# PaddleCV-SIG/MedicalSeg

Measured on AMD Instinct MI355X. Metric: 3D-voxels/sec fwd+bwd, VNet 128^3 fp32, higher is better.
Workload: dtype f32

## Files before the change

### medicalseg_amd/csrc/msk_common.h

```cpp
#pragma once
#include <hip/hip_runtime.h>
#include <hip/hip_ext.h>

#include <cstdint>
#include <cstdio>
#include <cstring>
#include <map>
#include <set>
#include <string>
#include <utility>
#include <vector>

#include "msegk.h"

struct msk_prof_entry {
  double total_ms = 0.0;
  long calls = 0;
};

struct msk_pending_event {
  hipEvent_t a, b;
  const char* tag;
};

// ... 4 lines not shown
  virtual int prepack(msk_ctx* ctx, const void* p, size_t bytes) = 0;
};

struct msk_ctx {
  int device = 0;
  hipStream_t stream = nullptr;
  std::string err;
  void* ws = nullptr;
  size_t ws_bytes = 0;
  void* ws2 = nullptr;
  size_t ws2_bytes = 0;
  void* ws3 = nullptr;
  size_t ws3_bytes = 0;
  long wbf_tin_groups = -1;
  long wbf_pad_min_voxels = 1L << 18;
  hipEvent_t t0 = nullptr, t1 = nullptr;
  hipEvent_t ev_xctx = nullptr;
  bool prof = false;
  std::map<std::string, msk_prof_entry> prof_map;
  std::vector<msk_pending_event> prof_pending;
  std::vector<hipEvent_t> event_pool;
  std::vector<hipEvent_t> marks;
  std::set<std::string> tag_pool;
  bool prof_shapes = false;
  int conv_impl = 0;
  bool no_winograd = false;
  bool wbf = true;
  bool dst_split_done = false;
  bool stats_fused = false;
  bool wgrad_db_done = false;
  bool xform_written = false;
  std::set<const void*> xform_ok;
  bool conv_fp16 = false;
  int wbf_tin_map = 1;
  int wbf_mr4 = 1;
  int wbf_variant = -1;
  int halo_tile = -1;
  int wgrad_chunk = -1;
  char prof_prefix[48] = {0};
  long wgrad_async_max_m = 0;
  float* scalar_ring = nullptr;
  int scalar_next = 0;
  long scalar_served = 0;
  float* scalar_ring_side = nullptr;
  int scalar_next_side = 0;
  long scalar_served_side = 0;
  int wbf_tpb = 0;
  msk_pack_cache* wpack = nullptr;
  int wbf_pack_cache = 1;
  msk_pack_cache* spack = nullptr;
  int wbf_pack_lds = 1;
  int wbf_bpf = 1;
  int wbf_fused_sh = 1;
  int wbf_gemm_form = -1;
  int wbf_ks_blocks = 2;
  int noop_after_merge = 0;
  int wgrad_c1_wpc = 2;
  int eager_tail_main = 1;
  int prof_paused = 0;
  int prof_attach = 1;
  int small_pack_cache = 1;
  int wbf_prepack = 1;
  int ks_legacy = 0;
  int wgrad_fork = 1;
  int wbf_fused_bl = 2;
  int wbf_fuse = 1;
  int conv_split = 2;
  int bwd_fuse = -1;
  int foldn_wgs = 0;
  int wgrad_wino_rounds = 0;
  int wgrad_rounds = 8;
  int poison = -1;
  hipStream_t side = nullptr;
  void* ws_side = nullptr;
  size_t ws_side_bytes = 0;
  void* ws3_side = nullptr;
  size_t ws3_side_bytes = 0;
  hipEvent_t ev_fork = nullptr, ev_join = nullptr;
  hipEvent_t ev_late = nullptr;
  bool late_valid = false;
  const float* late_ptr = nullptr;
  size_t late_count = 0;
  float* late_alpha = nullptr;
  struct { float* param = nullptr; const float* grad = nullptr; float* velocity = nullptr; size_t count = 0;
           float lr = 0, momentum = 0, weight_decay = 0, grad_scale = 0; } late_piece;
  int late_split = 1;
  bool wgrad_async = false;
  bool side_dirty = false;
  hipEvent_t fork_event = nullptr;
  int fork_attach = 1;
  bool fork_recorded = false;
  void* stage[2] = {nullptr, nullptr};
  size_t stage_bytes[2] = {0, 0};
  hipEvent_t stage_ev[2] = {nullptr, nullptr};
  int stage_next = 0;
  void* comm = nullptr;
  void* comm_grad = nullptr;
  hipStream_t comm_stream = nullptr;
  hipEvent_t ev_comm_main = nullptr, ev_comm_side = nullptr, ev_comm_done = nullptr, ev_comm_back = nullptr;
  int c1_h2 = 1;
  int dst_split = 1;
  int wgrad_reduce_rows = 1;
  int ks_stats = 1;
  int ks_lds = 1;
  int ks_nr_max = 4;
  int wgrad_lds_pad = 0;
// ... 134 lines not shown
```

### medicalseg_amd/csrc/msk_conv_wbf.hip

```cpp
#include <type_traits>
#include "msk_pack.h"
#include "msk_wbf.h"
#ifndef WBF_TIN_SYNC
#define WBF_TIN_SYNC 1
#endif

#ifndef WBF_PROBE
#define WBF_PROBE 0
#endif
typedef _Float16 f16x8 __attribute__((ext_vector_type(8)));
typedef _Float16 f16x2 __attribute__((ext_vector_type(2)));

namespace {

constexpr int nxi_of(int K) { return K == 5 ? 8 : 6; }

__device__ __forceinline__ void split3_one(float x, unsigned short& hi, unsigned short& mid, unsigned short& lo) {
  hi = __builtin_bit_cast(unsigned short, (__bf16)x);
  const float r = x - __uint_as_float((unsigned)hi << 16);
  mid = __builtin_bit_cast(unsigned short, (__bf16)r);
  const float r2 = r - __uint_as_float((unsigned)mid << 16);
  lo = __builtin_bit_cast(unsigned short, (__bf16)r2);
}
__device__ __forceinline__ unsigned pack_f16_pair(float a, float b) {
// ... 566 lines not shown
    }
    if (WY) {
#pragma unroll
      for (int q = 0; q < 2; ++q) {
        float wx[8], wy[8], wz[8], ww[8];
#pragma unroll
        for (int j = 0; j < 4; ++j) {
          const float4 e = win[PADW + j][q];
          wx[j] = e.x; wy[j] = e.y; wz[j] = e.z; ww[j] = e.w;
        }
#pragma unroll
        for (int j = 4; j < 8; ++j) wx[j] = wy[j] = wz[j] = ww[j] = 0.f;
        tin_transform<1, K>(wx, v[q * 4 + 0]);
        tin_transform<1, K>(wy, v[q * 4 + 1]);
        tin_transform<1, K>(wz, v[q * 4 + 2]);
        tin_transform<1, K>(ww, v[q * 4 + 3]);
      }
#pragma unroll
      for (int xi = 0; xi < NXI; ++xi) store_xi<K, NP>(yb2 + t * tstep + (long)xi * b.y_xi, plane, v, xi, sc2);
    }
#pragma unroll
    for (int j = 0; j < KEEP; ++j) {
      win[j][0] = win[j + 4][0];
      win[j][1] = win[j + 4][1];
    }
#pragma unroll
    for (int j = 0; j < 4; ++j) {
      win[KEEP + j][0] = nxt[j][0];
      win[KEEP + j][1] = nxt[j][1];
    }
  }
  }
  if (want_cmax) wbf_cmax_commit(b.y_cmax, cg, cmx, true);
}

struct GemmArgs {
  const char* V;
  const char* U;
  float* M;
  int N, T, KC, CN, LD, LH, DP, HP;
  int tiles_d, tiles_h, ngrp, ksplit, kc_per;
  int tpb, nblk;
  long v_xi, v_plane;
  long u_xi;
  long m_xi;
};

__device__ __forceinline__ uint4 buf_load16(__amdgpu_buffer_rsrc_t r, unsigned lane_bytes, unsigned uniform_bytes) {
  return __builtin_bit_cast(uint4, __builtin_amdgcn_raw_buffer_load_b128(r, (int)lane_bytes, (int)uniform_bytes, 0));
}

typedef int i32x4 __attribute__((ext_vector_type(4)));
__device__ __forceinline__ void wbf_dma16(i32x4 rs, unsigned lds_addr, unsigned voff, unsigned soff) {
  asm volatile("s_mov_b32 m0, %0\n\ts_nop 0\n\tbuffer_load_dwordx4 %1, %2, %3 offen lds" ::"s"(lds_addr), "v"(voff), "s"(rs), "s"(soff) : "memory");
}

#define WBF_MFMA(acc, av, bv) \
  acc = __builtin_amdgcn_mfma_f32_32x32x16_bf16(__builtin_bit_cast(bf16x8, av), __builtin_bit_cast(bf16x8, bv), acc, 0, 0, 0)
#define WBF_MFMA_H(acc, av, bv) \
  acc = __builtin_amdgcn_mfma_f32_32x32x16_f16(__builtin_bit_cast(f16x8, av), __builtin_bit_cast(f16x8, bv), acc, 0, 0, 0)

template <int TH>
__device__ __forceinline__ void frag_pos(int r, int& a, int& b) {
  if (TH == 16) {
    if (r < 4) { a = 0; b = r; }
    else if (r < 12) { a = 0; b = r + 4; }
    else if (r < 16) { a = 0; b = r - 8; }
    else if (r < 20) { a = 1; b = r - 4; }
    else if (r < 28) { a = 1; b = r - 16; }
    else { a = 1; b = r - 28; }
  } else if (TH == 8) {
    if (r < 4) { a = 0; b = r; }
    else if (r < 12) { a = 1; b = r - 4; }
    else if (r < 16) { a = 0; b = r - 8; }
    else if (r < 20) { a = 3; b = r - 16; }
    else if (r < 28) { a = 2; b = r - 20; }
    else { a = 3; b = r - 24; }
  } else {
    a = r / TH;
    b = r % TH;
  }
}

template <int TH>
__device__ __forceinline__ void subfrag_pos(int g, int r, int& d, int& h) {
  if (TH == 8) { d = (g >> 1) * 4 + (g & 1) + 2 * (r >> 3); h = r & 7; }
  else { d = g / (TH / 16); h = (g % (TH / 16)) * 16 + r; }
}
#define WBF_MFMA16_H(acc, wv, av) \
  acc = __builtin_amdgcn_mfma_f32_16x16x32_f16(__builtin_bit_cast(f16x8, wv), __builtin_bit_cast(f16x8, av), acc, 0, 0, 0)

template <int MR, int WM, int WN, int TD, int TH, int K, int NP, int BPF = 1, int SH = 32>
__global__ void __launch_bounds__(WM * WN * 64)
wbf_gemm_k(GemmArgs a) {
  static_assert((WM * WN == 4 || WM * WN == 2) && WM * MR * 32 == TD * TH, "tile shape");
  static_assert(SH == 32 || (SH == 16 && NP == 2 && BPF == 1), "stage form");
  constexpr int CPS = SH == 16 ? 2 : 1;
  constexpr int NT = WM * WN * 64;
  constexpr int NXI = nxi_of(K), T2 = K * K, PADK = (K - 1) / 2;
  constexpr int HDt = TD + K - 1, HPt = TH + K - 1, NSLOT = HDt * HPt, NPL = 2 * NP, NIT = CPS * NPL * NSLOT, ROUNDS = (NIT + NT - 1) / NT;
  static_assert(SH == 32 || NSLOT % 16 == 0, "planes of the image start on a bank row (subfrag_pos)");
  __shared__ uint4 lds[ROUNDS * NT];

  const int tid = threadIdx.x;
  const int wave = __builtin_amdgcn_readfirstlane(tid >> 6), lane = tid & 63, li = lane & 31, lh = lane >> 5;
  const int wm = wave / WN, wn = wave % WN;

// ... 236 lines not shown

struct FusedArgs {
  GemmArgs g;
  float* dst;
  int dld;
  long dvn;
  int dvd, dvh, dvw;
  const float* bias;
  const float* prelu;
  int accumulate;
  const float* in_amax;
  const float* w_amax;
  int scaled;
  float* stat_partial;
  int per_xcd;
  int LW;
  float* st_lo;
  float* st_hi;
  int csplit;
  const float* acc_src;
};

struct WfRec {
  float n, mean, m2;
};
__device__ __forceinline__ WfRec wfrec_merge(WfRec a, WfRec b) {
  if (b.n == 0.f) return a;
  if (a.n == 0.f) return b;
  WfRec r;
  r.n = a.n + b.n;
  const float d = b.mean - a.mean, f = b.n / r.n;
  r.mean = a.mean + d * f;
  r.m2 = a.m2 + b.m2 + d * d * a.n * f;
  return r;
}

template <int K>
__device__ __forceinline__ void at_column(int xi, float& c0, float& c1, float& c2, float& c3) {
  const int last = K == 5 ? 7 : 5;
  c0 = xi == last ? 0.f : 1.f;
  if (xi == 0) { c1 = c2 = c3 = 0.f; return; }
  if (xi == last) { c1 = c2 = 0.f; c3 = 1.f; return; }
  const float sg = (xi & 1) ? 1.f : -1.f;
  const int pr = (xi - 1) >> 1;
  const float p = pr == 0 ? 1.f : (pr == 1 ? 2.f : 0.5f);
  c1 = sg * p;
  c2 = p * p;
  c3 = sg * p * p * p;
}

#ifndef WBF_FUSED_BPF
#define WBF_FUSED_BPF 3
#endif
template <int MR, int WM, int WN, int TD, int TH, int K, int NP, bool STATS, int BPF = (NP == 2 ? WBF_FUSED_BPF : 1), int BL = 0, int SH = 32>
__global__ void __launch_bounds__(WM * WN * 64, 2)
wbf_gemm_fused_k(FusedArgs f) {
  static_assert(WM * WN == 4 && WM * MR * 32 == TD * TH, "tile shape");
  static_assert(SH == 32 || (SH == 16 && BL == 2 && WN == 1 && NP == 2), "16x16x32: pipelined form, one column fragment");
  constexpr int NS16 = 2 * MR;
  const GemmArgs& a = f.g;
  constexpr int NT = WM * WN * 64;
  constexpr int NXI = nxi_of(K), T2 = K * K, PADK = (K - 1) / 2;
  constexpr int HDt = TD + K - 1, HPt = TH + K - 1, NSLOT = HDt * HPt, NPL = 2 * NP, NIT = NPL * NSLOT, ROUNDS = (NIT + NT - 1) / NT;
  constexpr int NBF = T2 * NP;
  constexpr int BROUNDS = (NBF + WM * WN - 1) / (WM * WN);
  static_assert(BL == 0 || NIT % 64 == 0, "weights through LDS: wave-granular tile");
  static_assert(BL != 1 || WN == 1, "B through LDS, whole stage: one column fragment");
  constexpr int PH = WN == 1 ? 4 : 5;
  constexpr int PQ_T[6] = {0, T2 * 1 / PH, T2 * 2 / PH, T2 * 3 / PH, PH > 4 ? T2 * 4 / PH : T2, T2};
  constexpr int PQ_FR = (T2 - PQ_T[PH - 1]) * NP * WN;
  constexpr int PQ_SLOT = PQ_FR * 64;
  static_assert(BL != 2 || (NP == 2 && WM * WN == 4 && WN <= 2 && PQ_T[1] * NP * WN >= 4), "pipelined form: fp16 x 2 pieces, four wavefronts");
  __shared__ uint4 lds[BL == 2 ? 2 * NIT + 2 * PQ_SLOT : (BL ? NIT + NBF * 64 : ROUNDS * NT)];

  const int tid = threadIdx.x;
  const int wave = __builtin_amdgcn_readfirstlane(tid >> 6), lane = tid & 63, li = lane & 31, lh = lane >> 5;
  const int wm = wave / WN, wn = wave % WN;

  int b = (blockIdx.x & 7) * f.per_xcd + (blockIdx.x >> 3);
  if ((int)(blockIdx.x >> 3) >= f.per_xcd || b >= a.nblk) return;
  const int tile_id = b;
  const int thi = b % a.tiles_h;
  b /= a.tiles_h;
  const int tdi = b % a.tiles_d;
  b /= a.tiles_d;
  const int t = b % a.T;
  const int n = b / a.T;

  unsigned voff[ROUNDS];
#pragma unroll
  for (int r = 0; r < ROUNDS; ++r) {
    int it = r * NT + tid;
    if (it >= NIT) it = 0;
    const int pk = it / NSLOT, slot = it - pk * NSLOT;
    const int row = slot / HPt, col = slot - row * HPt;
    voff[r] = (unsigned)(pk * a.v_plane + ((long)row * a.HP + col) * 16);
  }
  const char* vtile0 = a.V + ((long)(n * a.T + t) * a.KC) * NPL * a.v_plane +
                       ((long)(tdi * TD + 2 - PADK) * a.HP + thi * TH + 2 - PADK) * 16;
  const unsigned ulane = (unsigned)(lh * a.CN + wn * 32 + li) * 16u;
  const unsigned ustep = (unsigned)a.CN * 32u;
  const unsigned uchunk = (unsigned)NP * ustep;
  const unsigned utap = (unsigned)a.KC * uchunk;

  int arow[MR];
#pragma unroll
  for (int mr = 0; mr < MR; ++mr) {
    int fa, fb;
    frag_pos<TH>(li, fa, fb);
    arow[mr] = lh * NSLOT + ((wm * MR + mr) * (32 / TH) + fa) * HPt + fb;
  }

  f32x16 yo[4][MR];
#pragma unroll
  for (int i = 0; i < 4; ++i)
#pragma unroll
    for (int mr = 0; mr < MR; ++mr)
#pragma unroll
      for (int j = 0; j < 16; ++j) yo[i][mr][j] = 0.f;
  f32x4 yo16[4][NS16][2];
#pragma unroll
  for (int i = 0; i < 4; ++i)
#pragma unroll
    for (int s = 0; s < NS16; ++s)
#pragma unroll
      for (int ct = 0; ct < 2; ++ct) yo16[i][s][ct] = f32x4{0.f, 0.f, 0.f, 0.f};
  const int l16 = lane & 15, kq = lane >> 4;

  if constexpr (BL == 2) {
    const unsigned lds0 = (unsigned)(unsigned long)(__attribute__((address_space(3))) void*)lds;
    const int NS = NXI * a.KC;
    const unsigned voff_last = (ROUNDS - 1) * NT + wave * 64 < NIT ? voff[ROUNDS - 1] : voff[ROUNDS - 2];
    const int r_last = (ROUNDS - 1) * NT + wave * 64 < NIT ? ROUNDS - 1 : ROUNDS - 2;
    auto rsrc_of = [](const char* p_) {
      const unsigned long pa = (unsigned long)p_;
      i32x4 r_ = {(int)__builtin_amdgcn_readfirstlane((unsigned)pa), (int)(__builtin_amdgcn_readfirstlane((unsigned)(pa >> 32)) & 0xffffu),
                  (int)0xFFFFFFF0u, 0x00020000};
      return r_;
    };
    auto fill_tile = [&](int s_) {
      const int xi_ = s_ / a.KC, kc_ = s_ - xi_ * a.KC;
      const i32x4 vr = rsrc_of(vtile0 + (long)xi_ * a.v_xi);
      const unsigned so = (unsigned)(kc_ * NPL * a.v_plane);
      const unsigned dst = lds0 + (unsigned)((s_ & 1) * NIT + wave * 64) * 16u;
#pragma unroll
      for (int r = 0; r < ROUNDS - 1; ++r) wbf_dma16(vr, dst + (unsigned)(r * NT) * 16u, voff[r], so);
      wbf_dma16(vr, dst + (unsigned)(r_last * NT) * 16u, voff_last, so);
    };
    auto fill_weights = [&](int s_, auto qc) {
      constexpr int q = decltype(qc)::value;
      constexpr int f0 = PQ_T[q] * NP * WN, nf = (PQ_T[q + 1] - PQ_T[q]) * NP * WN, rounds = (nf + 3) / 4;
      const int xi_ = s_ / a.KC, kc_ = s_ - xi_ * a.KC;
      const i32x4 ur = rsrc_of(a.U + (long)xi_ * a.u_xi);
      const unsigned ukc = (unsigned)kc_ * uchunk;
#pragma unroll
      for (int r = 0; r < rounds; ++r) {
        int fr = r * 4 + wave;
        if (fr >= nf) fr -= 4;
        const int fg = (f0 + fr) / WN, fw = (f0 + fr) % WN;
        wbf_dma16(ur, lds0 + (unsigned)(2 * NIT + ((q + (s_ & PH & 1)) & 1) * PQ_SLOT + fr * 64) * 16u, (unsigned)(lh * a.CN + fw * 32 + li) * 16u,
                  (unsigned)(fg / NP) * utap + ukc + (unsigned)(fg % NP) * ustep);
      }
    };
    f32x16 acc[MR];
    int abase[MR];
    auto run_phase = [&](int s_, auto qc) {
      constexpr int q = decltype(qc)::value;
      constexpr int T0 = PQ_T[q], T1 = PQ_T[q + 1];
      const bool more = s_ + 1 < NS;
      if (q == 1 && more) asm volatile("s_waitcnt vmcnt(%0)" ::"n"(ROUNDS) : "memory");
      else asm volatile("s_waitcnt vmcnt(0)" ::: "memory");
      __builtin_amdgcn_s_barrier();
      asm volatile("" ::: "memory");
      if constexpr (q < PH - 1) fill_weights(s_, std::integral_constant<int, q + 1>{});
      else if (more) fill_weights(s_ + 1, std::integral_constant<int, 0>{});
      if (q == 0 && more) fill_tile(s_ + 1);
      const uint4* bl = lds + 2 * NIT + ((q + (s_ & PH & 1)) & 1) * PQ_SLOT + wn * 64 + lane;
      uint4 aq[2][MR][NP], bq[2][NP];
#pragma unroll
      for (int p = 0; p < NP; ++p) bq[T0 & 1][p] = bl[p * WN * 64];
#pragma unroll
      for (int mr = 0; mr < MR; ++mr) {
        const uint4* ap = lds + abase[mr] + (T0 / K) * HPt + (T0 % K);
#pragma unroll
        for (int p = 0; p < NP; ++p) aq[T0 & 1][mr][p] = ap[p * 2 * NSLOT];
      }
#pragma unroll
      for (int tap = T0; tap < T1; ++tap) {
        const int cur = tap & 1, nx = cur ^ 1;
        if (tap + 1 < T1) {
#pragma unroll
          for (int p = 0; p < NP; ++p) bq[nx][p] = bl[((tap + 1 - T0) * NP + p) * WN * 64];
#pragma unroll
          for (int mr = 0; mr < MR; ++mr) {
            const uint4* ap = lds + abase[mr] + ((tap + 1) / K) * HPt + ((tap + 1) % K);
#pragma unroll
            for (int p = 0; p < NP; ++p) aq[nx][mr][p] = ap[p * 2 * NSLOT];
          }
        }
        __builtin_amdgcn_sched_barrier(0);
        const uint4 bdown = wbf_hi_down(bq[cur][0]);
#pragma unroll
        for (int mr = 0; mr < MR; ++mr) WBF_MFMA_H(acc[mr], aq[cur][mr][NP - 1], bdown);
#pragma unroll
        for (int mr = 0; mr < MR; ++mr) WBF_MFMA_H(acc[mr], aq[cur][mr][0], bq[cur][NP - 1]);
#pragma unroll
        for (int mr = 0; mr < MR; ++mr) WBF_MFMA_H(acc[mr], aq[cur][mr][0], bq[cur][0]);
        __builtin_amdgcn_sched_barrier(0);
      }
    };
    f32x4 acc16[NS16][2];
    int arow16[NS16], abase16[NS16];
#pragma unroll
    for (int s = 0; s < NS16; ++s) {
      int dd, hh;
      subfrag_pos<TH>(wm * NS16 + s, l16, dd, hh);
      arow16[s] = (kq & 1) * NSLOT + dd * HPt + hh;
    }
    auto run_phase16 = [&](int s_, auto qc) {
      constexpr int q = decltype(qc)::value;
      constexpr int T0 = PQ_T[q], T1 = PQ_T[q + 1], NPAIR = (T1 - T0 + 1) / 2;
      const bool more = s_ + 1 < NS;
      if (q == 1 && more) asm volatile("s_waitcnt vmcnt(%0)" ::"n"(ROUNDS) : "memory");
      else asm volatile("s_waitcnt vmcnt(0)" ::: "memory");
      __builtin_amdgcn_s_barrier();
      asm volatile("" ::: "memory");
      if constexpr (q < PH - 1) fill_weights(s_, std::integral_constant<int, q + 1>{});
      else if (more) fill_weights(s_ + 1, std::integral_constant<int, 0>{});
      if (q == 0 && more) fill_tile(s_ + 1);
      const uint4* bl = lds + 2 * NIT + ((q + (s_ & PH & 1)) & 1) * PQ_SLOT + (kq & 1) * 32 + l16;
      const uint4* blk = bl + (kq >> 1) * NP * 64;
      const bool up = (kq >> 1) != 0;
      uint4 aq[2][NP], bq[2][2][NP], bdown[2];
      auto load_b = [&](int j, uint4 (&d_)[2][NP]) {
        const bool full = T0 + 2 * j + 1 < T1;
#pragma unroll
        for (int ct = 0; ct < 2; ++ct)
#pragma unroll
          for (int p = 0; p < NP; ++p) {
            if (full) {
              d_[ct][p] = blk[(2 * j * NP + p) * 64 + ct * 16];
            } else {
              const uint4 v = bl[(2 * j * NP + p) * 64 + ct * 16];
              d_[ct][p] = up ? uint4{0u, 0u, 0u, 0u} : v;
            }
          }
      };
      auto load_a = [&](int j, int sf, uint4 (&d_)[NP]) {
        const int t0 = T0 + 2 * j, t1 = t0 + 1 < T1 ? t0 + 1 : t0;
        const int off = up ? (t1 / K) * HPt + (t1 % K) : (t0 / K) * HPt + (t0 % K);
        const uint4* ap = lds + abase16[sf] + off;
#pragma unroll
        for (int p = 0; p < NP; ++p) d_[p] = ap[p * 2 * NSLOT];
      };
      load_b(0, bq[0]);
      load_a(0, 0, aq[0]);
#pragma unroll
      for (int it = 0; it < NS16 * NPAIR; ++it) {
        const int j = it / NS16, sf = it % NS16, cur = it & 1, nx = cur ^ 1, bcur = j & 1;
        if (sf == 0 && j + 1 < NPAIR) load_b(j + 1, bq[bcur ^ 1]);
        if (it + 1 < NS16 * NPAIR) load_a((it + 1) / NS16, (it + 1) % NS16, aq[nx]);
        __builtin_amdgcn_sched_barrier(0);
        if (sf == 0) {
#pragma unroll
          for (int ct = 0; ct < 2; ++ct) bdown[ct] = wbf_hi_down(bq[bcur][ct][0]);
        }
#pragma unroll
        for (int ct = 0; ct < 2; ++ct) WBF_MFMA16_H(acc16[sf][ct], aq[cur][NP - 1], bdown[ct]);
#pragma unroll
        for (int ct = 0; ct < 2; ++ct) WBF_MFMA16_H(acc16[sf][ct], aq[cur][0], bq[bcur][ct][NP - 1]);
#pragma unroll
        for (int ct = 0; ct < 2; ++ct) WBF_MFMA16_H(acc16[sf][ct], aq[cur][0], bq[bcur][ct][0]);
        __builtin_amdgcn_sched_barrier(0);
      }
    };
    fill_weights(0, std::integral_constant<int, 0>{});
    fill_tile(0);
    if constexpr (SH == 16) {
#pragma unroll 1
    for (int s_ = 0; s_ < NS; ++s_) {
      const int xi = s_ / a.KC, kc = s_ - xi * a.KC;
      if (kc == 0) {
#pragma unroll
        for (int s = 0; s < NS16; ++s)
#pragma unroll
          for (int ct = 0; ct < 2; ++ct) acc16[s][ct] = f32x4{0.f, 0.f, 0.f, 0.f};
      }
#pragma unroll
      for (int s = 0; s < NS16; ++s) abase16[s] = arow16[s] + (s_ & 1) * NIT;
      run_phase16(s_, std::integral_constant<int, 0>{});
      run_phase16(s_, std::integral_constant<int, 1>{});
      run_phase16(s_, std::integral_constant<int, 2>{});
      run_phase16(s_, std::integral_constant<int, 3>{});
      if (kc == a.KC - 1) {
        float c0, c1, c2, c3;
        at_column<K>(xi, c0, c1, c2, c3);
#pragma unroll
        for (int s = 0; s < NS16; ++s)
#pragma unroll
          for (int ct = 0; ct < 2; ++ct)
#pragma unroll
            for (int j = 0; j < 4; ++j) {
              const float m = acc16[s][ct][j];
              yo16[0][s][ct][j] = fmaf(c0, m, yo16[0][s][ct][j]);
              yo16[1][s][ct][j] = fmaf(c1, m, yo16[1][s][ct][j]);
              yo16[2][s][ct][j] = fmaf(c2, m, yo16[2][s][ct][j]);
              yo16[3][s][ct][j] = fmaf(c3, m, yo16[3][s][ct][j]);
            }
      }
    }
    } else {
#pragma unroll 1
    for (int s_ = 0; s_ < NS; ++s_) {
      const int xi = s_ / a.KC, kc = s_ - xi * a.KC;
      if (kc == 0) {
#pragma unroll
        for (int mr = 0; mr < MR; ++mr)
#pragma unroll
          for (int j = 0; j < 16; ++j) acc[mr][j] = 0.f;
      }
#pragma unroll
      for (int mr = 0; mr < MR; ++mr) abase[mr] = arow[mr] + (s_ & 1) * NIT;
      run_phase(s_, std::integral_constant<int, 0>{});
      run_phase(s_, std::integral_constant<int, 1>{});
      run_phase(s_, std::integral_constant<int, 2>{});
      run_phase(s_, std::integral_constant<int, 3>{});
      if constexpr (PH > 4) run_phase(s_, std::integral_constant<int, 4>{});
      if (kc == a.KC - 1) {
        float c0, c1, c2, c3;
        at_column<K>(xi, c0, c1, c2, c3);
#pragma unroll
        for (int mr = 0; mr < MR; ++mr)
#pragma unroll
          for (int j = 0; j < 16; ++j) {
            const float m = acc[mr][j];
            yo[0][mr][j] = fmaf(c0, m, yo[0][mr][j]);
            yo[1][mr][j] = fmaf(c1, m, yo[1][mr][j]);
            yo[2][mr][j] = fmaf(c2, m, yo[2][mr][j]);
            yo[3][mr][j] = fmaf(c3, m, yo[3][mr][j]);
          }
      }
    }
    }
    __syncthreads();
  } else {
#pragma unroll 1
// ... 144 lines not shown
#pragma unroll
          for (int mr = 0; mr < MR; ++mr) WBF_MFMA(acc[mr], aq[cur][mr][0], bq[bcur][NP / 2]);
#pragma unroll
          for (int mr = 0; mr < MR; ++mr) WBF_MFMA(acc[mr], aq[cur][mr][0], bq[bcur][0]);
        } else if (NP == 2 && (WBF_PROBE & 16)) {
#pragma unroll
          for (int mr = 0; mr < MR; ++mr)
#pragma unroll
            for (int p = 0; p < NP; ++p)
              asm volatile("" ::"v"(aq[cur][mr][p].x), "v"(aq[cur][mr][p].y), "v"(aq[cur][mr][p].z), "v"(aq[cur][mr][p].w),
                           "v"(bq[bcur][p].x), "v"(bq[bcur][p].y), "v"(bq[bcur][p].z), "v"(bq[bcur][p].w));
        } else if (NP == 2) {
          const uint4 bdown = wbf_hi_down(bq[bcur][0]);
#pragma unroll
          for (int mr = 0; mr < MR; ++mr) WBF_MFMA_H(acc[mr], aq[cur][mr][NP - 1], bdown);
#pragma unroll
          for (int mr = 0; mr < MR; ++mr) WBF_MFMA_H(acc[mr], aq[cur][mr][0], bq[bcur][NP - 1]);
#pragma unroll
          for (int mr = 0; mr < MR; ++mr) WBF_MFMA_H(acc[mr], aq[cur][mr][0], bq[bcur][0]);
        } else {
#pragma unroll
          for (int mr = 0; mr < MR; ++mr) WBF_MFMA_H(acc[mr], aq[cur][mr][0], bq[bcur][0]);
        }
        __builtin_amdgcn_sched_barrier(0);
      }
      }
    }
    float c0, c1, c2, c3;
    at_column<K>(xi, c0, c1, c2, c3);
#pragma unroll
    for (int mr = 0; mr < MR; ++mr)
#pragma unroll
      for (int j = 0; j < 16; ++j) {
        const float m = acc[mr][j];
        yo[0][mr][j] = fmaf(c0, m, yo[0][mr][j]);
        yo[1][mr][j] = fmaf(c1, m, yo[1][mr][j]);
        yo[2][mr][j] = fmaf(c2, m, yo[2][mr][j]);
        yo[3][mr][j] = fmaf(c3, m, yo[3][mr][j]);
      }
  }

  }
  if constexpr (SH == 16) {
    const wbf_unscale osc = f.scaled ? wbf_unscale_of(wbf_scale_of(f.in_amax), wbf_scale_of(f.w_amax)) : wbf_unscale{1.f, 1.f};
    const long vox0 = ((long)n * f.dvn + (long)(4 * t) * f.dvw) * f.dld;
    const long wst = (long)f.dvw * f.dld;
    const bool split_st = f.st_lo != nullptr;
    const long swst = split_st ? (wst >> 1) : wst;
    const long aoff = f.acc_src ? (f.acc_src - f.dst) : 0;
    const int wlim = f.LW - 4 * t;
    WfRec rec[2];
#pragma unroll
    for (int ct = 0; ct < 2; ++ct) {
      const int co = ct * 16 + l16;
      const float bv = f.bias ? f.bias[co] : 0.f;
      const float sl = f.prelu ? f.prelu[co] : 1.f;
      float* obase = f.dst + vox0 + co;
      float* sbase = split_st ? (co < f.csplit ? f.st_lo + co : f.st_hi + (co - f.csplit)) + (vox0 >> 1) : obase;
      float sk = 0.f, s1 = 0.f, s2 = 0.f, cnt = 0.f;
#pragma unroll
      for (int s = 0; s < NS16; ++s) {
        float* op[4];
        bool ok[4];
#pragma unroll
        for (int jj = 0; jj < 4; ++jj) {
          int dd, hh;
          subfrag_pos<TH>(wm * NS16 + s, 4 * kq + jj, dd, hh);
          const int d = tdi * TD + dd, h = thi * TH + hh;
          ok[jj] = d < a.LD && h < a.LH;
          op[jj] = obase + ((long)d * f.dvd + (long)h * f.dvh) * f.dld;
        }
        float old[4][4];
        if (f.accumulate) {
#pragma unroll
          for (int jj = 0; jj < 4; ++jj)
#pragma unroll
            for (int i = 0; i < 4; ++i) old[jj][i] = (ok[jj] && i < wlim) ? __builtin_nontemporal_load(op[jj] + aoff + i * wst) : 0.f;
        }
#pragma unroll
        for (int jj = 0; jj < 4; ++jj) {
          if (!ok[jj]) continue;
#pragma unroll
          for (int i = 0; i < 4; ++i) {
            if (i >= wlim) break;
            float r = fmaf(yo16[i][s][ct][jj] * osc.r0, osc.r1, bv);
            if (f.accumulate) r += old[jj][i];
            if (f.prelu) r = r > 0.f ? r : sl * r;
            if (split_st) sbase[((op[jj] - obase) >> 1) + i * swst] = r;
            else op[jj][i * wst] = r;
            if (STATS) {
              if (cnt == 0.f) sk = r;
              const float dlt = r - sk;
              s1 += dlt;
              s2 = fmaf(dlt, dlt, s2);
              cnt += 1.f;
            }
          }
        }
      }
      rec[ct] = WfRec{0.f, 0.f, 0.f};
      if (STATS && cnt > 0.f) {
        rec[ct].n = cnt;
        rec[ct].mean = sk + s1 / cnt;
        rec[ct].m2 = fmaxf(s2 - s1 * s1 / cnt, 0.f);
      }
    }
    if (STATS) {
#pragma unroll
      for (int ct = 0; ct < 2; ++ct) {
        WfRec w = rec[ct], o;
        o.n = __shfl_xor(w.n, 16, 64);
        o.mean = __shfl_xor(w.mean, 16, 64);
        o.m2 = __shfl_xor(w.m2, 16, 64);
        w = (kq & 1) == 0 ? wfrec_merge(w, o) : wfrec_merge(o, w);
        o.n = __shfl_xor(w.n, 32, 64);
        o.mean = __shfl_xor(w.mean, 32, 64);
        o.m2 = __shfl_xor(w.m2, 32, 64);
        rec[ct] = (kq & 2) == 0 ? wfrec_merge(w, o) : wfrec_merge(o, w);
      }
      __syncthreads();
      float* sh = reinterpret_cast<float*>(lds);
      if (kq == 0) {
#pragma unroll
        for (int ct = 0; ct < 2; ++ct) {
          float* p_ = sh + (wave * 32 + ct * 16 + l16) * 3;
          p_[0] = rec[ct].n; p_[1] = rec[ct].mean; p_[2] = rec[ct].m2;
        }
      }
      __syncthreads();
      if (wm == 0 && kq == 0) {
#pragma unroll
        for (int ct = 0; ct < 2; ++ct) {
          WfRec r = rec[ct];
#pragma unroll
          for (int q = 1; q < WM; ++q) {
            const float* p_ = sh + (q * 32 + ct * 16 + l16) * 3;
            WfRec e = {p_[0], p_[1], p_[2]};
            r = wfrec_merge(r, e);
          }
          float* g_ = f.stat_partial + ((long)tile_id * a.CN + ct * 16 + l16) * 3;
          g_[0] = r.n; g_[1] = r.mean; g_[2] = r.m2;
        }
      }
    }
    return;
  }
  const int co = wn * 32 + li;
  const wbf_unscale osc = f.scaled ? wbf_unscale_of(wbf_scale_of(f.in_amax), wbf_scale_of(f.w_amax)) : wbf_unscale{1.f, 1.f};
  const float bv = f.bias ? f.bias[co] : 0.f;
  const float sl = f.prelu ? f.prelu[co] : 1.f;
  float* obase = f.dst + ((long)n * f.dvn + (long)(4 * t) * f.dvw) * f.dld + co;
  const long wst = (long)f.dvw * f.dld;
  const bool split_st = f.st_lo != nullptr;
  float* sbase = split_st ? (co < f.csplit ? f.st_lo + co : f.st_hi + (co - f.csplit)) + (((long)n * f.dvn + (long)(4 * t) * f.dvw) * f.dld >> 1) : obase;
  const long swst = split_st ? (wst >> 1) : wst;
  const long aoff = f.acc_src ? (f.acc_src - f.dst) : 0;
  const int wlim = f.LW - 4 * t;
  float sk = 0.f, s1 = 0.f, s2 = 0.f, cnt = 0.f;
#pragma unroll
  for (int mr = 0; mr < MR; ++mr) {
#pragma unroll
    for (int jq = 0; jq < 4; ++jq) {
      float* op[4];
      bool ok[4];
#pragma unroll
      for (int jj = 0; jj < 4; ++jj) {
        int fa, fb;
        frag_pos<TH>(jj + 8 * jq + 4 * lh, fa, fb);
        const int d = tdi * TD + (wm * MR + mr) * (32 / TH) + fa, h = thi * TH + fb;
        ok[jj] = d < a.LD && h < a.LH;
        op[jj] = obase + ((long)d * f.dvd + (long)h * f.dvh) * f.dld;
      }
      float old[4][4];
      if (f.accumulate) {
#pragma unroll
        for (int jj = 0; jj < 4; ++jj)
#pragma unroll
          for (int i = 0; i < 4; ++i) old[jj][i] = (ok[jj] && i < wlim) ? __builtin_nontemporal_load(op[jj] + aoff + i * wst) : 0.f;
      }
#pragma unroll
      for (int jj = 0; jj < 4; ++jj) {
        if (!ok[jj]) continue;
#pragma unroll
        for (int i = 0; i < 4; ++i) {
          if (i >= wlim) break;
          float r = fmaf(yo[i][mr][jq * 4 + jj] * osc.r0, osc.r1, bv);
          if (f.accumulate) r += old[jj][i];
          if (f.prelu) r = r > 0.f ? r : sl * r;
          if ((WBF_PROBE & 8) && r != 12345.678f) continue;
          if (split_st) sbase[((op[jj] - obase) >> 1) + i * swst] = r;
          else op[jj][i * wst] = r;
          if (STATS) {
            if (cnt == 0.f) sk = r;
// ... 346 lines not shown
    WbfPackList l{};
    long most = 0;
    for (int r : which) {
      const WbfPackRow& e = row(r);
      if (e.K != kc[0] || e.NP != kc[1]) continue;
      l.row[l.n++] = (unsigned char)r;
      const long blocks = ((long)e.K * e.K * e.d.KC * 16 * e.d.CN + 255) / 256;
      if (blocks > most) most = blocks;
    }
    if (l.n == 0) continue;
    bool lds_ok = ctx->wbf_pack_lds != 0;
    long most_lds = 0;
    for (int i = 0; i < l.n && lds_ok; ++i) {
      const WbfPackDesc& dd = row(l.row[i]).d;
      lds_ok = dd.CK == dd.KC * 16 && dd.CN % 8 == 0 && dd.B % 4 == 0 && (((uintptr_t)dd.w) & 15) == 0 &&
               (dd.swap ? dd.B >= dd.CK : dd.B >= dd.CN);
      const long blocks = (long)dd.KC * (dd.CN / 8);
      if (blocks > most_lds) most_lds = blocks;
    }
    if (lds_ok) {
      if (most_lds > 4L * ctx->num_cu) most_lds = 4L * ctx->num_cu;
      const dim3 grid((unsigned)most_lds, (unsigned)l.n);
      if (one) l.n = -1;
      const size_t lds = (size_t)128 * kc[0] * kc[0] * kc[0] * sizeof(float);
      msk_launch_scope ls(ctx, "wbf_pack_weights");
      if (kc[0] == 5 && kc[1] == 2) hipLaunchKernelGGL((wbf_pack_weights_lds_k<5, 2>), grid, dim3(256), lds, ctx->stream, table, l, single);
      else if (kc[0] == 5) hipLaunchKernelGGL((wbf_pack_weights_lds_k<5, 3>), grid, dim3(256), lds, ctx->stream, table, l, single);
      else if (kc[1] == 2) hipLaunchKernelGGL((wbf_pack_weights_lds_k<3, 2>), grid, dim3(256), lds, ctx->stream, table, l, single);
      else if (kc[1] == 3) hipLaunchKernelGGL((wbf_pack_weights_lds_k<3, 3>), grid, dim3(256), lds, ctx->stream, table, l, single);
      else hipLaunchKernelGGL((wbf_pack_weights_lds_k<3, 1>), grid, dim3(256), lds, ctx->stream, table, l, single);
      MSK_LAUNCH_CHECK(ctx);
      continue;
    }
    if (most > 8L * ctx->num_cu) most = 8L * ctx->num_cu;
    const dim3 grid((unsigned)most, (unsigned)l.n);
    if (one) l.n = -1;
    msk_launch_scope ls(ctx, "wbf_pack_weights");
    if (kc[0] == 5 && kc[1] == 2) hipLaunchKernelGGL((wbf_pack_weights_k<5, 2>), grid, dim3(256), 0, ctx->stream, table, l, single);
    else if (kc[0] == 5) hipLaunchKernelGGL((wbf_pack_weights_k<5, 3>), grid, dim3(256), 0, ctx->stream, table, l, single);
    else if (kc[1] == 2) hipLaunchKernelGGL((wbf_pack_weights_k<3, 2>), grid, dim3(256), 0, ctx->stream, table, l, single);
    else if (kc[1] == 3) hipLaunchKernelGGL((wbf_pack_weights_k<3, 3>), grid, dim3(256), 0, ctx->stream, table, l, single);
    else hipLaunchKernelGGL((wbf_pack_weights_k<3, 1>), grid, dim3(256), 0, ctx->stream, table, l, single);
    MSK_LAUNCH_CHECK(ctx);
  }
  for (int r : which)
    if (r != kScratch) rows.e[r].valid = true;
  return 0;
}

template <int MR, int WM, int WN, int TD, int TH, int K, int NP>
void launch_fused(msk_ctx* ctx, const char* tag, const FusedArgs& fa, bool stats, bool fork) {
  const dim3 grid((unsigned)(8 * fa.per_xcd));
  constexpr int NITc = 2 * NP * (TD + K - 1) * (TH + K - 1);
  if constexpr (WN == 2 && WM == 2 && NP == 2 && NITc % 64 == 0) {
    if (ctx->wbf_fused_bl == 2 && fa.g.CN == 64) {
      if (stats) MSK_LAUNCH_TIMED_F(ctx, tag, fork, (wbf_gemm_fused_k<MR, WM, WN, TD, TH, K, NP, true, 1, 2>), grid, dim3(WM * WN * 64), 0, fa);
      else MSK_LAUNCH_TIMED_F(ctx, tag, fork, (wbf_gemm_fused_k<MR, WM, WN, TD, TH, K, NP, false, 1, 2>), grid, dim3(WM * WN * 64), 0, fa);
      return;
    }
  }
  if constexpr (WN == 1 && NP == 2 && NITc % 64 == 0) {
    if (ctx->wbf_fused_bl == 2 && fa.g.CN == 32 && ctx->wbf_fused_sh != 0) {
      if (stats) MSK_LAUNCH_TIMED_F(ctx, tag, fork, (wbf_gemm_fused_k<MR, WM, WN, TD, TH, K, NP, true, 1, 2, 16>), grid, dim3(WM * WN * 64), 0, fa);
      else MSK_LAUNCH_TIMED_F(ctx, tag, fork, (wbf_gemm_fused_k<MR, WM, WN, TD, TH, K, NP, false, 1, 2, 16>), grid, dim3(WM * WN * 64), 0, fa);
      return;
    }
    if (ctx->wbf_fused_bl == 2 && fa.g.CN == 32) {
      if (stats) MSK_LAUNCH_TIMED_F(ctx, tag, fork, (wbf_gemm_fused_k<MR, WM, WN, TD, TH, K, NP, true, 1, 2>), grid, dim3(WM * WN * 64), 0, fa);
      else MSK_LAUNCH_TIMED_F(ctx, tag, fork, (wbf_gemm_fused_k<MR, WM, WN, TD, TH, K, NP, false, 1, 2>), grid, dim3(WM * WN * 64), 0, fa);
      return;
    }
    if (ctx->wbf_fused_bl && fa.g.CN == 32) {
      if (stats) MSK_LAUNCH_TIMED_F(ctx, tag, fork, (wbf_gemm_fused_k<MR, WM, WN, TD, TH, K, NP, true, 1, 1>), grid, dim3(WM * WN * 64), 0, fa);
      else MSK_LAUNCH_TIMED_F(ctx, tag, fork, (wbf_gemm_fused_k<MR, WM, WN, TD, TH, K, NP, false, 1, 1>), grid, dim3(WM * WN * 64), 0, fa);
      return;
    }
  }
  if (stats) MSK_LAUNCH_TIMED_F(ctx, tag, fork, (wbf_gemm_fused_k<MR, WM, WN, TD, TH, K, NP, true>), grid, dim3(WM * WN * 64), 0, fa);
  else MSK_LAUNCH_TIMED_F(ctx, tag, fork, (wbf_gemm_fused_k<MR, WM, WN, TD, TH, K, NP, false>), grid, dim3(WM * WN * 64), 0, fa);
}
template <int K, int NP>
void launch_fused_variant(msk_ctx* ctx, const char* tag, int variant, const FusedArgs& fa, bool stats, bool fork) {
  switch (variant) {
    case 3: launch_fused<2, 1, 4, 8, 8, K, NP>(ctx, tag, fa, stats, fork); break;
    case 4: launch_fused<2, 4, 1, 16, 16, K, NP>(ctx, tag, fa, stats, fork); break;
    default: launch_fused<2, 2, 2, 8, 16, K, NP>(ctx, tag, fa, stats, fork); break;
  }
}

template <int K, int NP>
int run_pipeline(msk_ctx* ctx, const GConv& g, const float* w_canon, int A, int B, int swap, const WbfGeom& geo, const Var* bv, bool dry) {
  constexpr int NXI = nxi_of(K), NPL = 2 * NP;
  const int TD = bv->TD, TH = bv->TH, variant = bv->id;
  const int* pm = geo.perm;
  const int LD = geo.LD, LH = geo.LH, LW = geo.LW;
  const int vstr[3] = {g.DH * g.DW, g.DW, 1};
  const int tstr[3] = {K * K, K, 1};
  const int T = geo.T, KC = g.CK / 16;
  const int tiles_d = (LD + TD - 1) / TD, tiles_h = (LH + TH - 1) / TH;
  const int DP = geo.DP, HP = geo.HP;
  const int WN = bv->WN;
  const int ngrp = g.CN / (WN * 32);

  const long base_blocks = (long)NXI * ngrp * tiles_h * tiles_d * T * g.N;
  int ksplit = 1, kc_per = KC;
  const int form = pick_gemm_form(ctx, WN, K, NP, KC);
// ... 44 lines not shown
    const bool cached = g.w_persistent && ctx->wbf_pack_cache != 0;
    int row;
    if (cached) {
      row = c->row_of(ctx, kr, NXI * u_xi);
      if (row < 0) return -1;
    } else {
      row = WbfPackCache::kScratch;
      key.out = (unsigned short*)msk_workspace2(ctx, NXI * u_xi);
      if (!key.out) return -1;
      key.amax = c->amax + (size_t)row * kWbfAmaxWays;
      c->scratch = kr;
    }
    if (!(cached && c->rows.e[row].valid) && c->build(ctx, std::vector<int>{row}) != 0) return -1;
    U = (char*)c->row(row).d.out;
    w_amax = c->row(row).d.amax;
  }
  const float* in_amax = nullptr;
  if (NP != 3) {
    if (g.fuse) in_amax = g.fuse->amax;
    else if (g.in_amax) in_amax = g.in_amax;
    else in_amax = msk_absmax(ctx, g.src, g.sld, g.ck_real > 0 ? g.ck_real : g.CK, (long)g.N * g.SD * g.SH * g.SW, g.xform ? (float*)g.xform : nullptr);
    if (!in_amax) return -1;
  }
  float* hdr_copy = (NP != 3 && g.xform && !g.fuse && in_amax != (const float*)g.xform) ? (float*)g.xform : nullptr;

  {
    WbfTinArgs ta{};
    ta.src = g.src; ta.sld = g.sld;
    ta.svn = (long)g.DD * g.DH * g.DW; ta.svd = vstr[pm[0]]; ta.svh = vstr[pm[1]]; ta.svw = vstr[pm[2]];
    ta.N = g.N; ta.LD = LD; ta.LH = LH; ta.LW = LW; ta.T = T; ta.CK = g.CK; ta.KC = KC;
    ta.DP = DP; ta.HP = HP; ta.V = V; ta.v_xi = (long)v_xi;
    ta.amax = in_amax;
    ta.amax_copy = hdr_copy;
    ta.c_real = g.ck_real;
    if (g.fuse) {
      if (msk_wbf_transform_dual(ctx, K, NP, ta, *g.fuse, true) != 0) return -1;
      if (g.fuse->Y && ctx->wgrad_async && ctx->side != nullptr && ctx->wgrad_fork == 0) {
        hipEventRecord(ctx->ev_fork, ctx->stream);
        ctx->fork_recorded = true;
      }
    } else if (msk_wbf_transform(ctx, 0, K, NP, ta) != 0) {
      return -1;
    }
  }
  const bool fork_after = g.fuse && g.fuse->Y && ctx->wgrad_async && ctx->side != nullptr && ctx->wgrad_fork == 1 && ctx->fork_attach != 0;
  GemmArgs ga{};
  ga.V = V; ga.U = U; ga.M = M;
  ga.N = g.N; ga.T = T; ga.KC = KC; ga.CN = g.CN; ga.LD = LD; ga.LH = LH; ga.DP = DP; ga.HP = HP;
  ga.tiles_d = tiles_d; ga.tiles_h = tiles_h; ga.ngrp = ngrp; ga.ksplit = ksplit; ga.kc_per = kc_per;
  ga.v_xi = (long)v_xi; ga.v_plane = (long)v_plane; ga.u_xi = (long)u_xi; ga.m_xi = (long)m_xi;
  const char* tag = NP == 3 ? "wbf_gemm_k" : (NP == 2 ? "wbf_gemm_h2_k" : "wbf_gemm_f16_k");
  if (ctx->prof && ctx->prof_shapes) {
    char buf[200];
    const bool sh16 = fuse_out && K == 5 && NP == 2 && variant == 4 && g.CN == 32 && ctx->wbf_fused_bl == 2 && ctx->wbf_fused_sh != 0;
    snprintf(buf, sizeof(buf), "%s[ck=%d,cn=%d,n=%d,dhw=%dx%dx%d,k=%d,ks=%d%s%s]", tag, g.CK, g.CN, g.N, g.DD, g.DH, g.DW, K, ksplit,
             fuse_out ? (sh16 ? ",fused,sh16" : ",fused") : "", fuse_out || form == 0 ? "" : ",form=2");
    tag = msk_intern_tag(ctx, buf);
  }
  if (fuse_out) {
    FusedArgs fa{};
    fa.g = ga;
    fa.g.nblk = (int)(base_blocks / NXI);
    fa.dst = g.dst; fa.dld = g.dld;
    fa.dvn = (long)g.DD * g.DH * g.DW; fa.dvd = vstr[pm[0]]; fa.dvh = vstr[pm[1]]; fa.dvw = vstr[pm[2]];
    fa.bias = g.bias; fa.prelu = g.prelu; fa.accumulate = g.accumulate;
    fa.acc_src = g.accumulate ? g.acc_src : nullptr;
    fa.in_amax = in_amax; fa.w_amax = w_amax; fa.scaled = NP != 3 ? 1 : 0;
    fa.stat_partial = SP;
    fa.per_xcd = (fa.g.nblk + 7) / 8;
    fa.LW = LW;
    if (g.dst_lo && g.dst_hi && g.dst_csplit > 0 && g.accumulate && g.dld == 2 * g.dst_csplit && g.CN == 2 * g.dst_csplit && !fuse_stats) {
      fa.st_lo = g.dst_lo; fa.st_hi = g.dst_hi; fa.csplit = g.dst_csplit;
      ctx->dst_split_done = true;
    }
    launch_fused_variant<K, NP>(ctx, tag, variant, fa, fuse_stats, fork_after);
    MSK_LAUNCH_CHECK(ctx);
    if (fuse_stats) {
      if (g.stats_ps) {
        const int tps = fa.g.nblk / g.N;
        for (int n = 0; n < g.N; ++n) {
          msk_bn_fin fn{};
          if (g.fin) {
            fn = *g.fin;
            const long o = (long)n * g.fin_stride;
            fn.save_mean += o; fn.save_invstd += o; fn.scale += o; fn.shift += o;
          }
          if (msk_bn_stats_merge(ctx, SP + (size_t)n * tps * g.CN * 3, tps, g.CN, g.stats + (size_t)n * 2 * g.CN, g.fin ? &fn : nullptr) != 0) return -1;
        }
      } else if (msk_bn_stats_merge(ctx, SP, fa.g.nblk, g.CN, g.stats, g.fin) != 0) {
        return -1;
      }
      ctx->stats_fused = true;
    }
    if (g.xform) ctx->xform_written = true;
    return 1;
  }
  launch_gemm_variant<K, NP>(ctx, tag, variant, ga, nblk, form);
  MSK_LAUNCH_CHECK(ctx);
  {
    ToutArgs oa{};
    oa.M = M; oa.m_xi = (long)m_xi; oa.ksplit = ksplit;
    oa.N = g.N; oa.T = T; oa.LD = LD; oa.LH = LH; oa.LW = LW; oa.CN = g.CN;
    oa.dst = g.dst; oa.dld = g.dld;
    oa.dvn = (long)g.DD * g.DH * g.DW; oa.dvd = vstr[pm[0]]; oa.dvh = vstr[pm[1]]; oa.dvw = vstr[pm[2]];
    oa.bias = g.bias; oa.prelu = g.prelu; oa.accumulate = g.accumulate;
    oa.acc_src = g.accumulate ? g.acc_src : nullptr;
    oa.stat_partial = SP;
// ... 148 lines not shown
```

### medicalseg_amd/csrc/msk_ctx.hip

```cpp
#include <cstdlib>

#include "msk_common.h"

thread_local std::string g_msk_global_err;

int msk_fail(msk_ctx* ctx, const char* file, int line, const char* what, const char* detail) {
  char buf[1024];
  const char* base = strrchr(file, '/');
  snprintf(buf, sizeof(buf), "%s:%d: %s: %s", base ? base + 1 : file, line, what, detail ? detail : "");
  if (ctx) ctx->err = buf;
  g_msk_global_err = buf;
  return -1;
}

static void* grow(msk_ctx* ctx, void** p, size_t* cur, size_t bytes) {
  if (bytes <= *cur) return *p;
  if (*p) {
    hipStreamSynchronize(ctx->stream);
    hipFree(*p);
    *p = nullptr;
    *cur = 0;
  }
  size_t want = bytes + (bytes >> 2);
  if (hipMalloc(p, want) != hipSuccess) {
// ... 406 lines not shown
  }
  if (strcmp(key, "wgrad_async_max_m") == 0) {
    ctx->wgrad_async_max_m = value;
    return 0;
  }
  if (strcmp(key, "wino_bf3") == 0) {
    ctx->wbf = value != 0;
    return 0;
  }
  if (strcmp(key, "conv_fp16") == 0) {
    ctx->conv_fp16 = value != 0;
    return 0;
  }
  if (strcmp(key, "wbf_tin_map") == 0) {
    ctx->wbf_tin_map = value;
    return 0;
  }
  if (strcmp(key, "wbf_mr4") == 0) {
    ctx->wbf_mr4 = value;
    return 0;
  }
  if (strcmp(key, "wbf_variant") == 0) {
    ctx->wbf_variant = value;
    return 0;
  }
  if (strcmp(key, "direct_conv") == 0) {
    ctx->no_winograd = value != 0;
    return 0;
  }
  if (strcmp(key, "wbf_tin_groups") == 0) {
    ctx->wbf_tin_groups = value;
    return 0;
  }
  if (strcmp(key, "wbf_pad_min_voxels") == 0) {
    ctx->wbf_pad_min_voxels = value > 0 ? value : 0;
    return 0;
  }
  if (strcmp(key, "wbf_pack_cache") == 0) {
    ctx->wbf_pack_cache = value;
    return 0;
  }
  if (strcmp(key, "wbf_pack_lds") == 0) {
    ctx->wbf_pack_lds = value;
    return 0;
  }
  if (strcmp(key, "wbf_bpf") == 0) {
    ctx->wbf_bpf = value;
    return 0;
  }
  if (strcmp(key, "wbf_fused_sh") == 0) {
    ctx->wbf_fused_sh = value != 0 ? 1 : 0;
    return 0;
  }
  if (strcmp(key, "wbf_gemm_form") == 0) {
    ctx->wbf_gemm_form = value == 0 || value == 2 ? value : -1;
    return 0;
  }
  if (strcmp(key, "wbf_ks_blocks") == 0) {
    ctx->wbf_ks_blocks = value > 0 ? value : 2;
    return 0;
  }
  if (strcmp(key, "wgrad_c1_wpc") == 0) {
    ctx->wgrad_c1_wpc = value < 1 ? 1 : value;
    return 0;
  }
  if (strcmp(key, "eager_tail_main") == 0) {
    ctx->eager_tail_main = value;
    return 0;
  }
  if (strcmp(key, "fork_attach") == 0) {
    ctx->fork_attach = value;
    return 0;
  }
  if (strcmp(key, "prof_paused") == 0) {
    ctx->prof_paused = value;
    return 0;
  }
  if (strcmp(key, "prof_attach") == 0) {
    ctx->prof_attach = value;
    return 0;
  }
  if (strcmp(key, "noop_after_merge") == 0) {
    ctx->noop_after_merge = value;
    return 0;
  }
  if (strcmp(key, "small_pack_cache") == 0) {
    ctx->small_pack_cache = value;
    return 0;
  }
  if (strcmp(key, "wbf_prepack") == 0) {
    ctx->wbf_prepack = value;
    return 0;
  }
  if (strcmp(key, "dp_mode") == 0) {
    if (value < 0 || value > 3 || (value == 2 && ctx->comm != nullptr && ctx->comm_grad == nullptr))
      return msk_fail(ctx, __FILE__, __LINE__, "msk_set_option", "dp_mode: 0, 1, 2 or 3 (2 only before msk_dp_init)");
    ctx->dp_mode = value;
    return 0;
  }
  if (strcmp(key, "ew_cap") == 0) {
    msk_set_ew_caps(value, 0);
    return 0;
  }
  if (strcmp(key, "dst_split") == 0) {
    ctx->dst_split = value;
    return 0;
// ... 140 lines not shown
```

Baseline: 249.7 million.

## Extend 16x16x32 MFMA pipelined fused Winograd GEMM to two column fragments

Generalises the 16x16x32 MFMA pipelined fused kernel from one column wavefront to WN=2, so CN=64 K=5 convolutions can use it. It adds a custom phase table that keeps whole tap pairs per phase, offsets B-fragment LDS indexing and output/stat channel indices by wn, and runs the fifth phase. A new ctx knob, on by default, selects this path. It also adds an m0 clobber to the LDS DMA asm and several static asserts. The aim is better MFMA utilisation and scheduling for the 64-channel 5x5 layers, at the risk of indexing mistakes and an uneven phase split.

New measurement: 250.0 million (median of 5 runs). About the same (+0.1%).

```diff
diff --git a/medicalseg_amd/csrc/msk_common.h b/medicalseg_amd/csrc/msk_common.h
--- a/medicalseg_amd/csrc/msk_common.h
+++ b/medicalseg_amd/csrc/msk_common.h
@@ -80,6 +80,7 @@
   int wbf_pack_lds = 1;
   int wbf_bpf = 1;
   int wbf_fused_sh = 1;
+  int wbf_fused_sh64 = 1;
   int wbf_gemm_form = -1;
   int wbf_ks_blocks = 2;
   int noop_after_merge = 0;
diff --git a/medicalseg_amd/csrc/msk_conv_wbf.hip b/medicalseg_amd/csrc/msk_conv_wbf.hip
--- a/medicalseg_amd/csrc/msk_conv_wbf.hip
+++ b/medicalseg_amd/csrc/msk_conv_wbf.hip
@@ -642,7 +642,7 @@
 
 typedef int i32x4 __attribute__((ext_vector_type(4)));
 __device__ __forceinline__ void wbf_dma16(i32x4 rs, unsigned lds_addr, unsigned voff, unsigned soff) {
-  asm volatile("s_mov_b32 m0, %0\n\ts_nop 0\n\tbuffer_load_dwordx4 %1, %2, %3 offen lds" ::"s"(lds_addr), "v"(voff), "s"(rs), "s"(soff) : "memory");
+  asm volatile("s_mov_b32 m0, %0\n\ts_nop 0\n\tbuffer_load_dwordx4 %1, %2, %3 offen lds" ::"s"(lds_addr), "v"(voff), "s"(rs), "s"(soff) : "memory", "m0");
 }
 
 #define WBF_MFMA(acc, av, bv) \
@@ -985,11 +985,24 @@
 #ifndef WBF_FUSED_BPF
 #define WBF_FUSED_BPF 3
 #endif
+struct WbfPhaseTab {
+  int t[6];
+};
+constexpr WbfPhaseTab wbf_phase_tab(int WN, int SH, int T2) {
+  if (WN == 1) return {{0, T2 * 1 / 4, T2 * 2 / 4, T2 * 3 / 4, T2, T2}};
+  if (SH == 16 && T2 == 25) return {{0, 6, 12, 16, 20, 25}};
+  return {{0, T2 * 1 / 5, T2 * 2 / 5, T2 * 3 / 5, T2 * 4 / 5, T2}};
+}
+constexpr int wbf_phase_max(const WbfPhaseTab& tb) {
+  int m = 0;
+  for (int q = 0; q < 5; ++q) m = tb.t[q + 1] - tb.t[q] > m ? tb.t[q + 1] - tb.t[q] : m;
+  return m;
+}
 template <int MR, int WM, int WN, int TD, int TH, int K, int NP, bool STATS, int BPF = (NP == 2 ? WBF_FUSED_BPF : 1), int BL = 0, int SH = 32>
 __global__ void __launch_bounds__(WM * WN * 64, 2)
 wbf_gemm_fused_k(FusedArgs f) {
   static_assert(WM * WN == 4 && WM * MR * 32 == TD * TH, "tile shape");
-  static_assert(SH == 32 || (SH == 16 && BL == 2 && WN == 1 && NP == 2), "16x16x32: pipelined form, one column fragment");
+  static_assert(SH == 32 || (SH == 16 && BL == 2 && WN <= 2 && NP == 2), "16x16x32: pipelined form");
   constexpr int NS16 = 2 * MR;
   const GemmArgs& a = f.g;
   constexpr int NT = WM * WN * 64;
@@ -1000,10 +1013,17 @@
   static_assert(BL == 0 || NIT % 64 == 0, "weights through LDS: wave-granular tile");
   static_assert(BL != 1 || WN == 1, "B through LDS, whole stage: one column fragment");
   constexpr int PH = WN == 1 ? 4 : 5;
-  constexpr int PQ_T[6] = {0, T2 * 1 / PH, T2 * 2 / PH, T2 * 3 / PH, PH > 4 ? T2 * 4 / PH : T2, T2};
-  constexpr int PQ_FR = (T2 - PQ_T[PH - 1]) * NP * WN;
+  constexpr WbfPhaseTab PQ_TAB = wbf_phase_tab(WN, SH, T2);
+  constexpr int PQ_T[6] = {PQ_TAB.t[0], PQ_TAB.t[1], PQ_TAB.t[2], PQ_TAB.t[3], PQ_TAB.t[4], PQ_TAB.t[5]};
+  constexpr int PQ_FR = wbf_phase_max(PQ_TAB) * NP * WN;
   constexpr int PQ_SLOT = PQ_FR * 64;
   static_assert(BL != 2 || (NP == 2 && WM * WN == 4 && WN <= 2 && PQ_T[1] * NP * WN >= 4), "pipelined form: fp16 x 2 pieces, four wavefronts");
+  static_assert(PQ_T[0] == 0 && PQ_T[PH] == T2 && PQ_T[5] == T2, "phase table covers the stage");
+  static_assert(SH != 16 || ((PQ_T[1] - PQ_T[0]) % 2 == 0 && (PQ_T[2] - PQ_T[1]) % 2 == 0 && (PQ_T[3] - PQ_T[2]) % 2 == 0 &&
+                             (PH == 4 || (PQ_T[4] - PQ_T[3]) % 2 == 0)), "16x16x32: whole tap pairs per phase");
+  static_assert(BL != 2 || WN != 2 || ((PQ_T[1] - PQ_T[0]) * NP * WN % 4 == 0 && (PQ_T[2] - PQ_T[1]) * NP * WN % 4 == 0 && (PQ_T[3] - PQ_T[2]) * NP * WN % 4 == 0 &&
+                                       (PQ_T[4] - PQ_T[3]) * NP * WN % 4 == 0 && (PQ_T[5] - PQ_T[4]) * NP * WN % 4 == 0), "whole fill rounds per phase");
+  static_assert(SH != 16 || NSLOT % 16 == 0, "planes of the tile image start on a bank row (subfrag_pos)");
   __shared__ uint4 lds[BL == 2 ? 2 * NIT + 2 * PQ_SLOT : (BL ? NIT + NBF * 64 : ROUNDS * NT)];
 
   const int tid = threadIdx.x;
@@ -1101,6 +1121,7 @@
       constexpr int q = decltype(qc)::value;
       constexpr int T0 = PQ_T[q], T1 = PQ_T[q + 1];
       const bool more = s_ + 1 < NS;
+      static_assert(ROUNDS < 64, "vmcnt is a 6-bit count");
       if (q == 1 && more) asm volatile("s_waitcnt vmcnt(%0)" ::"n"(ROUNDS) : "memory");
       else asm volatile("s_waitcnt vmcnt(0)" ::: "memory");
       __builtin_amdgcn_s_barrier();
@@ -1161,8 +1182,8 @@
       if constexpr (q < PH - 1) fill_weights(s_, std::integral_constant<int, q + 1>{});
       else if (more) fill_weights(s_ + 1, std::integral_constant<int, 0>{});
       if (q == 0 && more) fill_tile(s_ + 1);
-      const uint4* bl = lds + 2 * NIT + ((q + (s_ & PH & 1)) & 1) * PQ_SLOT + (kq & 1) * 32 + l16;
-      const uint4* blk = bl + (kq >> 1) * NP * 64;
+      const uint4* bl = lds + 2 * NIT + ((q + (s_ & PH & 1)) & 1) * PQ_SLOT + wn * 64 + (kq & 1) * 32 + l16;
+      const uint4* blk = bl + (kq >> 1) * NP * WN * 64;
       const bool up = (kq >> 1) != 0;
       uint4 aq[2][NP], bq[2][2][NP], bdown[2];
       auto load_b = [&](int j, uint4 (&d_)[2][NP]) {
@@ -1172,9 +1193,9 @@
 #pragma unroll
           for (int p = 0; p < NP; ++p) {
             if (full) {
-              d_[ct][p] = blk[(2 * j * NP + p) * 64 + ct * 16];
+              d_[ct][p] = blk[(2 * j * NP + p) * WN * 64 + ct * 16];
             } else {
-              const uint4 v = bl[(2 * j * NP + p) * 64 + ct * 16];
+              const uint4 v = bl[(2 * j * NP + p) * WN * 64 + ct * 16];
               d_[ct][p] = up ? uint4{0u, 0u, 0u, 0u} : v;
             }
           }
@@ -1225,6 +1246,7 @@
       run_phase16(s_, std::integral_constant<int, 1>{});
       run_phase16(s_, std::integral_constant<int, 2>{});
       run_phase16(s_, std::integral_constant<int, 3>{});
+      if constexpr (PH > 4) run_phase16(s_, std::integral_constant<int, 4>{});
       if (kc == a.KC - 1) {
         float c0, c1, c2, c3;
         at_column<K>(xi, c0, c1, c2, c3);
@@ -1475,7 +1497,7 @@
     WfRec rec[2];
 #pragma unroll
     for (int ct = 0; ct < 2; ++ct) {
-      const int co = ct * 16 + l16;
+      const int co = wn * 32 + ct * 16 + l16;
       const float bv = f.bias ? f.bias[co] : 0.f;
       const float sl = f.prelu ? f.prelu[co] : 1.f;
       float* obase = f.dst + vox0 + co;
@@ -1557,11 +1579,11 @@
           WfRec r = rec[ct];
 #pragma unroll
           for (int q = 1; q < WM; ++q) {
-            const float* p_ = sh + (q * 32 + ct * 16 + l16) * 3;
+            const float* p_ = sh + ((q * WN + wn) * 32 + ct * 16 + l16) * 3;
             WfRec e = {p_[0], p_[1], p_[2]};
             r = wfrec_merge(r, e);
           }
-          float* g_ = f.stat_partial + ((long)tile_id * a.CN + ct * 16 + l16) * 3;
+          float* g_ = f.stat_partial + ((long)tile_id * a.CN + wn * 32 + ct * 16 + l16) * 3;
           g_[0] = r.n; g_[1] = r.mean; g_[2] = r.m2;
         }
       }
@@ -2014,6 +2036,13 @@
 void launch_fused(msk_ctx* ctx, const char* tag, const FusedArgs& fa, bool stats, bool fork) {
   const dim3 grid((unsigned)(8 * fa.per_xcd));
   constexpr int NITc = 2 * NP * (TD + K - 1) * (TH + K - 1);
+  if constexpr (WN == 2 && WM == 2 && NP == 2 && K == 5 && NITc % 64 == 0) {
+    if (ctx->wbf_fused_bl == 2 && fa.g.CN == 64 && ctx->wbf_fused_sh64 != 0) {
+      if (stats) MSK_LAUNCH_TIMED_F(ctx, tag, fork, (wbf_gemm_fused_k<MR, WM, WN, TD, TH, K, NP, true, 1, 2, 16>), grid, dim3(WM * WN * 64), 0, fa);
+      else MSK_LAUNCH_TIMED_F(ctx, tag, fork, (wbf_gemm_fused_k<MR, WM, WN, TD, TH, K, NP, false, 1, 2, 16>), grid, dim3(WM * WN * 64), 0, fa);
+      return;
+    }
+  }
   if constexpr (WN == 2 && WM == 2 && NP == 2 && NITc % 64 == 0) {
     if (ctx->wbf_fused_bl == 2 && fa.g.CN == 64) {
       if (stats) MSK_LAUNCH_TIMED_F(ctx, tag, fork, (wbf_gemm_fused_k<MR, WM, WN, TD, TH, K, NP, true, 1, 2>), grid, dim3(WM * WN * 64), 0, fa);
@@ -2164,7 +2193,8 @@
   const char* tag = NP == 3 ? "wbf_gemm_k" : (NP == 2 ? "wbf_gemm_h2_k" : "wbf_gemm_f16_k");
   if (ctx->prof && ctx->prof_shapes) {
     char buf[200];
-    const bool sh16 = fuse_out && K == 5 && NP == 2 && variant == 4 && g.CN == 32 && ctx->wbf_fused_bl == 2 && ctx->wbf_fused_sh != 0;
+    const bool sh16 = fuse_out && K == 5 && NP == 2 && ctx->wbf_fused_bl == 2 &&
+                      ((variant == 4 && g.CN == 32 && ctx->wbf_fused_sh != 0) || (variant == 5 && g.CN == 64 && ctx->wbf_fused_sh64 != 0));
     snprintf(buf, sizeof(buf), "%s[ck=%d,cn=%d,n=%d,dhw=%dx%dx%d,k=%d,ks=%d%s%s]", tag, g.CK, g.CN, g.N, g.DD, g.DH, g.DW, K, ksplit,
              fuse_out ? (sh16 ? ",fused,sh16" : ",fused") : "", fuse_out || form == 0 ? "" : ",form=2");
     tag = msk_intern_tag(ctx, buf);
diff --git a/medicalseg_amd/csrc/msk_ctx.hip b/medicalseg_amd/csrc/msk_ctx.hip
--- a/medicalseg_amd/csrc/msk_ctx.hip
+++ b/medicalseg_amd/csrc/msk_ctx.hip
@@ -482,6 +482,10 @@
     ctx->wbf_fused_sh = value != 0 ? 1 : 0;
     return 0;
   }
+  if (strcmp(key, "wbf_fused_sh64") == 0) {
+    ctx->wbf_fused_sh64 = value != 0 ? 1 : 0;
+    return 0;
+  }
   if (strcmp(key, "wbf_gemm_form") == 0) {
     ctx->wbf_gemm_form = value == 0 || value == 2 ? value : -1;
     return 0;
```
